# noisystreet/aither

Hardware: AMD Instinct MI355X
Metric: Mcell-updates/sec per iteration (residual+LU-SGS), 256^3 block; % HBM roofline (higher is better)
Workload: dtype f64

## Files before the change

aither_amd/csrc/agx_api.hip:

```cpp
#include "agx_kernels.hpp"
#include "agx_geometry.hpp"
#include "agx_mem.hpp"
#include <rccl/rccl.h>
#include <cstdarg>
#include <cstdio>
#include <cstring>
#include <cstdlib>
#include <cmath>
#include <vector>
#include <string>
#include <algorithm>

using namespace agx;

static char g_err[512] = "";
static int fail(const char* fmt, ...) {
  va_list ap;
  va_start(ap, fmt);
  vsnprintf(g_err, sizeof g_err, fmt, ap);
  va_end(ap);
  return 1;
}
#define HIPCHK(call)                                                       \
  do {                                                                     \
    hipError_t e_ = (call);                                                \
    if (e_ != hipSuccess)                                                  \
      return fail("%s failed: %s (%s:%d)", #call, hipGetErrorString(e_),   \
                  __FILE__, __LINE__);                                     \
  } while (0)
#define AGX_BY_MODE(sp, kernel, grid, block, stream, ...)                                  \
  do {                                                                                     \
    switch (agx::solver_mode_of(sp)) {                                                     \
      case 0: hipLaunchKernelGGL(kernel<0>, grid, block, 0, stream, __VA_ARGS__); break;   \
      case 1: hipLaunchKernelGGL(kernel<1>, grid, block, 0, stream, __VA_ARGS__); break;   \
      default: hipLaunchKernelGGL(kernel<2>, grid, block, 0, stream, __VA_ARGS__); break;  \
    }                                                                                      \
  } while (0)

namespace {

struct SweepGraphs {
  hipGraphExec_t g[2][2][2] = {};
  SweepGraphs() = default;
  SweepGraphs(SweepGraphs&& o) noexcept { memcpy(g, o.g, sizeof g); memset(o.g, 0, sizeof g); }
  ~SweepGraphs() { drop(); }
  hipGraphExec_t& at(bool forward, bool full, bool un_is_u) { return g[forward][full][un_is_u]; }
  void drop() {
    for (auto& g1 : g) for (auto& g2 : g1) for (auto& g3 : g2)
      if (g3) { hipGraphExecDestroy(g3); g3 = nullptr; }
  }
};

struct Block {
  BlockDev d;
  int global_pos = 0;
  DevBuf<double> slab;
  DevBuf<double> d2;
  DevBuf<double> blockmat;
  DevBuf<double> sweep_rec;
  bool sweep_geo_built = false;
  bool x_planes_current = false;
  DevBuf<double> mg_forcing, mg_mres, mg_xsave, mg_nodes;
// ... 64 lines not shown
  DevBuf<NormPartial> partials;
  long n_partials = 0;
  DevBuf<NormPartial> norm_out;
  PinnedBuf<NormPartial> norm_host;
  DevBuf<int> err_dev;
  PinnedBuf<int> err_host;
  DevBuf<double> halo_buf;
  DevBuf<double> stage_buf;
  DevBuf<double> rans_rec;
  bool use_gather = false;
  bool use_tile = true;
  int num_cu = 256;
  bool eager_ghosts = true;
  bool overlap = true;
  hipStream_t ov_stream = nullptr;
  hipEvent_t ov_ready = nullptr, ov_done = nullptr;
  bool visc_gather = false;
  bool visc_march = false;
  int lusgs_mode = 1;
  int spin_limit = 4000000;
  bool allow_fuse = true;
  bool fused_pending = false;
  bool use_graphs = true;
  bool sweep_records = true;
  bool sweep_three = true;
  hipStream_t cap_stream = nullptr;
  std::vector<hipStream_t> branch_streams;
  std::vector<hipEvent_t> branch_events;
  bool sweep_all_launch = true;
  DevBuf<BlockDev> blocks_tab;
  PinnedBuf<BlockDev> blocks_tab_host;
  SweepGraphs sweep_graph_all;
  bool mg_coarse = false;
  bool mres_plane_form = false;
  bool sweep_pipe = true;
  DevBuf<PipeJob> pipe_jobs[2];
  DevBuf<int> pipe_slot0;
  DevBuf<long long> pipe_progress;
  DevBuf<unsigned long long> pipe_ticket;
  size_t pipe_nblocks = 0;
  int pipe_njobs = 0, pipe_maxsteps = 0, pipe_waves = 4;
  long long pipe_launches = 0;
  bool halo_batch = true;
  bool halo_batch_required = false;
  int halo_batch_sides = 0;
  long halo_batch_nmax = 0;
  std::vector<int> halo_conn_order;
  struct HaloLevel { int first, sides; long nmax; };
  std::vector<HaloLevel> halo_levels;
  DevBuf<HaloSide> halo_tab_dev[5][2][2];
  bool halo_tab_valid[5][2] = {};
  int halo_set[5] = {};
  PinnedBuf<HaloSide> halo_tab_host;
  int mresid_split = 1;
  bool mresid_march = true;
  bool have_time_n = false;
  bool have_wall_data = false;
  bool in_iterate = false, ghosts_prefilled = false;
  bool mres_deferred = false;
  hipEvent_t norm_event = nullptr;
  bool consn_pending = false;
  bool state_is_time_n = false;
  long fused_parts = 0;
  bool timing = false;
  std::vector<std::pair<hipEvent_t, hipEvent_t>> ev_pool;
  std::vector<std::pair<int, int>> ev_used;
  double t_ms[G_NGROUP] = {};
  long t_n[G_NGROUP] = {};
};

static int my_side(const agx_ctx* c, const Conn& k);

namespace {

void resolve_timing(agx_ctx* c);

struct Timer {
  agx_ctx* c;
  int slot = -1;
  Timer(agx_ctx* ctx, int g) : c(ctx) {
    if (!c->timing) return;
    if (c->ev_used.size() >= 8192) resolve_timing(c);
    slot = (int)c->ev_used.size();
    if (slot >= (int)c->ev_pool.size()) {
      hipEvent_t a, b;
      if (hipEventCreate(&a) != hipSuccess || hipEventCreate(&b) != hipSuccess) {
        slot = -1;
        return;
      }
      c->ev_pool.emplace_back(a, b);
    }
    c->ev_used.emplace_back(g, slot);
    hipEventRecord(c->ev_pool[slot].first, c->stream);
  }
  ~Timer() {
    if (slot >= 0) hipEventRecord(c->ev_pool[slot].second, c->stream);
  }
};

void resolve_timing(agx_ctx* c) {
  if (c->ev_used.empty()) return;
  hipStreamSynchronize(c->stream);
  for (auto& u : c->ev_used) {
    float ms = 0.f;
    if (hipEventElapsedTime(&ms, c->ev_pool[u.second].first,
                            c->ev_pool[u.second].second) == hipSuccess) {
// ... 150 lines not shown
}

int halo_in_d2(const Block& b, int what) { return what == AGX_HALO_UPDATE && b.d.d2.base ? 1 : 0; }
void x_changed(agx_ctx* c) {
  for (auto& blk : c->blocks) blk.x_planes_current = false;
}
Planes5 halo_planes(Block& b, int what) {
  Planes5 r;
  r.rec = what == AGX_HALO_UPDATE ? b.d.sw_dyn : nullptr;
  const bool z2 = halo_in_d2(b, what) != 0;
  r.stride = z2 ? 2 : 1;
#if AGX_NEQ == 7
  if (what == AGX_HALO_TURB) {
    for (int e = 0; e < AGX_NEQ; ++e) r.p[e] = b.d.turb3[e < 3 ? e : 2];
    return r;
  }
#endif
  if (what == AGX_HALO_VELGRAD_A || what == AGX_HALO_VELGRAD_B) {
    for (int e = 0; e < AGX_NEQ; ++e) {
      const int comp = what == AGX_HALO_VELGRAD_A ? e : std::min(5 + e, 8);
      r.p[e] = b.d.vg + (long)comp * b.d.nplane;
    }
    return r;
  }
  for (int e = 0; e < AGX_NEQ; ++e)
    r.p[e] = what == AGX_HALO_STATE ? b.d.state[e]
             : (z2 ? b.d.d2.base + 2L * (PA_X + (e >> 1)) * b.d.d2.nd2 + (e & 1) : b.d.x[e]);
  return r;
}

int check_device_error(agx_ctx* c) {
  int* const err_host = c->err_host.get();
  if (*err_host) {
    const int code = *err_host;
    *err_host = 0;
    hipMemsetAsync(c->err_dev.get(), 0, sizeof(int), c->stream);
    if (code == 3)
      return fail("Singular matrix in Gauss-Jordan elimination!");
    if (code == AGX_ERR_TPG_ENERGY)
      return fail("thermallyPerfect: the temperature of a cell's specific energy was not "
                  "found (Newton's method did not converge in %d steps, or the energy lies "
                  "below the heat of formation)", AGX_TPG_NEWTON_MAX);
    if (code == 2) {
      c->pipe_nblocks = 0;
      return fail("LU-SGS pipeline: a k-plane waited beyond the spin limit for its "
                  "predecessor (AGX_LUSGS=plane / AGX_SWEEP_PIPE=0 select the "
                  "launch-per-hyperplane forms)");
    }
    return fail("a boundary-condition variant outside this build's coverage was requested");
  }
  return 0;
}

struct MarchPlan { dim3 grid; int kchunk; long nparts; };
int g_march_tj = 6;
bool tile_ok(const agx_ctx* c, const BlockDev& b) {
  return AGX_FAST && c->use_tile && !c->use_gather && (double)b.nplane * 8.0 < 4294967296.0;
}
bool all_tile_ok(const agx_ctx* c) {
  for (const auto& blk : c->blocks)
    if (!tile_ok(c, blk.d)) return false;
  return true;
}
MarchPlan march_plan(const agx_ctx* c, const BlockDev& b) {
  MarchPlan p;
  const int gx = (b.ni + 63) / 64, gy = (b.nj + g_march_tj - 1) / g_march_tj;
  if (tile_ok(c, b)) {
    const long steps = (long)gx * gy * b.nk;
    long np = std::min<long>(c->num_cu, std::max<long>(1, steps / 8));
    if (np >= 8) np -= np % 8;
    p.kchunk = 0;
    p.grid = dim3((unsigned)np);
    p.nparts = np;
    return p;
  }
  int nz = std::max(1, (int)std::lround(2048.0 / (gx * gy)));
  nz = std::min(nz, std::max(1, b.nk / 4));
  p.kchunk = (b.nk + nz - 1) / nz;
  nz = (b.nk + p.kchunk - 1) / p.kchunk;
  p.grid = dim3(gx, gy, nz);
  p.nparts = (long)gx * gy * nz;
  return p;
}

SlabDev make_slab(const BlockDev& b) {
  SlabDev sd;
  sd.base = b.vol - (long)PL_VOL * b.nplane;
  sd.nplane = b.nplane; sd.sx = b.sx; sd.sxy = b.sxy;
  sd.ni = b.ni; sd.nj = b.nj; sd.nk = b.nk; sd.ng = b.ng; sd.ioff = b.ioff;
  sd.st = (int)((b.state[0] - sd.base) / b.nplane);
  sd.sn = (int)((b.state2[0] - sd.base) / b.nplane);
  return sd;
}
template <int RECON, int LIM, int FLUX>
void launch_inv_kernel(agx_ctx* c, const BlockDev& b, double cfl, bool fuse,
                       const MarchArgs& ma, const MarchPlan& mp) {
  const SlabDev sd = make_slab(b);
  if (c->use_gather || AGX_NEQ != 5) {
    hipLaunchKernelGGL((k_inv_residual<RECON, LIM, FLUX>), cell_grid(b, CELL_BLOCK),
                       CELL_BLOCK, 0, c->stream, b, c->gas, c->sp, cfl);
    return;
  }
  const dim3 tb(64, g_march_tj + 2);
#if AGX_FAST
  if (tile_ok(c, b)) {
    if (fuse && ma.store_consn)
      hipLaunchKernelGGL((k_residual_tile<RECON, LIM, FLUX, 2, 6>), mp.grid, tb, 0,
                         c->stream, sd, c->gas, c->sp, cfl, ma);
    else if (fuse)
      hipLaunchKernelGGL((k_residual_tile<RECON, LIM, FLUX, 1, 6>), mp.grid, tb, 0,
                         c->stream, sd, c->gas, c->sp, cfl, ma);
    else
      hipLaunchKernelGGL((k_residual_tile<RECON, LIM, FLUX, 0, 6>), mp.grid, tb, 0,
                         c->stream, sd, c->gas, c->sp, cfl, ma);
  } else
#endif
  {
    if (fuse)
      hipLaunchKernelGGL((k_residual_march<RECON, LIM, FLUX, true, 6>), mp.grid, tb, 0,
                         c->stream, sd, c->gas, c->sp, cfl, ma);
    else
      hipLaunchKernelGGL((k_residual_march<RECON, LIM, FLUX, false, 6>), mp.grid, tb, 0,
                         c->stream, sd, c->gas, c->sp, cfl, ma);
  }
}
template <int RECON, int LIM>
// ... 829 lines not shown
  }
#if AGX_FAST
  for (auto& b : c->blocks)
    if (b.d.d2.base) {
      const long n = (long)b.d.d2.Pi * b.d.d2.Pj * (b.d.nk + 2 * b.d.ng);
      hipLaunchKernelGGL(k_d2_geo, dim3((n + 255) / 256), dim3(256), 0, c->stream, b.d);
    }
  HIPCHK(hipGetLastError());
#endif
  HIPCHK(hipStreamSynchronize(c->stream));
  for (auto& b : c->blocks) {
    b.fcen.reset();
    b.nodes_dev.reset();
  }
  return 0;
}
}

extern "C" {

const char* agx_last_error(void) { return g_err; }
const char* agx_version(void) {
#if AGX_TPG
  return "aither_gfx950 0.1 (HIP, gfx950, thermallyPerfect)";
#else
  return "aither_gfx950 0.1 (HIP, gfx950)";
#endif
}

int agx_ctx_create(int device, int rank, agx_ctx** out) {
  int ndev = 0;
  hipError_t e = hipGetDeviceCount(&ndev);
  if (e != hipSuccess || ndev <= 0)
    return fail("no HIP device available (%s): the gfx950 library has no CPU "
                "path", hipGetErrorString(e));
  if (device < 0 || device >= ndev) return fail("device %d out of range", device);
  HIPCHK(hipSetDevice(device));
  agx_ctx* c = new agx_ctx();
  c->device = device;
  c->rank = rank;
  if (const char* kn = getenv("AGX_KERNEL")) {
    c->use_gather = !strcmp(kn, "gather");
    c->use_tile = !strcmp(kn, "tile");
  }
  c->allow_fuse = !(getenv("AGX_NO_FUSE") && atoi(getenv("AGX_NO_FUSE")) != 0);
  {
    int ncu = 0;
    HIPCHK(hipDeviceGetAttribute(&ncu, hipDeviceAttributeMultiprocessorCount, device));
    if (ncu > 0) c->num_cu = ncu;
    if (const char* w = getenv("AGX_WORKGROUPS")) c->num_cu = std::max(1, atoi(w));
    if (const char* w = getenv("AGX_VISC")) {
      c->visc_gather = !strcmp(w, "gather");
      c->visc_march = !strcmp(w, "march");
    }
    if (const char* w = getenv("AGX_EAGER_GHOSTS")) c->eager_ghosts = atoi(w) != 0;
    if (const char* w = getenv("AGX_OVERLAP")) c->overlap = atoi(w) != 0;
    if (const char* w = getenv("AGX_LUSGS")) c->lusgs_mode = !strcmp(w, "plane") ? 0 : 1;
    if (const char* w = getenv("AGX_SPIN_LIMIT")) c->spin_limit = std::max(1, atoi(w));
    if (const char* w = getenv("AGX_GRAPHS")) c->use_graphs = atoi(w) != 0;
    if (const char* w = getenv("AGX_SWEEP_ALL")) c->sweep_all_launch = atoi(w) != 0;
    if (const char* w = getenv("AGX_SWEEP_PIPE")) c->sweep_pipe = atoi(w) != 0;
    if (const char* w = getenv("AGX_SWEEP_THREE")) c->sweep_three = atoi(w) != 0;
    if (const char* w = getenv("AGX_SWEEP_RECORDS")) c->sweep_records = atoi(w) != 0;
    if (const char* w = getenv("AGX_MRESID_SPLIT")) c->mresid_split = std::min(64, std::max(1, atoi(w)));
    if (const char* w = getenv("AGX_MRESID")) c->mresid_march = strcmp(w, "plane") != 0;
    if (const char* w = getenv("AGX_HALO_BATCH")) {
      c->halo_batch = strcmp(w, "0") != 0;
      c->halo_batch_required = !strcmp(w, "require");
    }
  }
  HIPCHK(c->err_dev.alloc(1));
  HIPCHK(hipMemset(c->err_dev.get(), 0, sizeof(int)));
  HIPCHK(c->err_host.alloc(1));
  *c->err_host.get() = 0;
  *out = c;
  return 0;
}

void agx_ctx_destroy(agx_ctx* c) {
  if (!c) return;
  hipSetDevice(c->device);
  hipStreamSynchronize(c->stream);
  if (c->nccl) ncclCommDestroy(c->nccl);
  for (auto& e : c->ev_pool) { hipEventDestroy(e.first); hipEventDestroy(e.second); }
  if (c->cap_stream) hipStreamDestroy(c->cap_stream);
  if (c->ov_stream) {
    hipStreamSynchronize(c->ov_stream);
    hipStreamDestroy(c->ov_stream);
    hipEventDestroy(c->ov_ready);
    hipEventDestroy(c->ov_done);
  }
  for (auto ev : c->branch_events) hipEventDestroy(ev);
  for (auto st : c->branch_streams) hipStreamDestroy(st);
  delete c;
}

int agx_ctx_set_stream(agx_ctx* c, void* s) {
  HIPCHK(hipSetDevice(c->device));
  HIPCHK(hipStreamSynchronize(c->stream));
  c->stream = (hipStream_t)s;
  return 0;
}

int agx_config_set(agx_ctx* c, const agx_config* cfg) {
  if (!c->blocks.empty())
    return fail("agx_config_set: the configuration is fixed after the first "
// ... 1042 lines not shown
  hipLaunchKernelGGL(k_mg_nodes, dim3((bc.d.ni + tb.x) / tb.x, (bc.d.nj + tb.y) / tb.y, bc.d.nk + 1),
                     tb, 0, cz->stream, bc.d, bc.mg_nodes.get());
  HIPCHK(hipGetLastError());
  if (mg_order(cz, f)) return 1;
  hipLaunchKernelGGL(k_mg_prolong, cell_grid(bf.d, tb), tb, 0, f->stream, bf.d, m,
                     (const double*)bc.mg_nodes.get(), bc.d.ni, bc.d.nj, bc.d.nk);
  mg_x_records(cz, bc);
  mg_x_records(f, bf);
  if (mg_x_from_planes(cz, bc) || mg_x_from_planes(f, bf)) return 1;
  HIPCHK(hipGetLastError());
  return 0;
}

int agx_store_time_n(agx_ctx* c, int also_nm1) {
  if (flush_consn(c)) return 1;
  c->have_time_n = true;
  for (auto& blk : c->blocks)
    if (blk.nr_max > 0) c->ghosts_prefilled = false;
  static const bool lazy = !(getenv("AGX_NO_LAZY_CONSN") && atoi(getenv("AGX_NO_LAZY_CONSN")));
  c->state_is_time_n = true;
  if (lazy && !also_nm1 && !c->use_gather && all_tile_ok(c)) { c->consn_pending = true; return 0; }
  for (auto& blk : c->blocks)
    hipLaunchKernelGGL(k_store_time_n, cell_grid(blk.d, CELL_BLOCK), CELL_BLOCK,
                       0, c->stream, blk.d, c->gas, also_nm1);
  HIPCHK(hipGetLastError());
  return 0;
}

int agx_phase_bc_faces(agx_ctx* c) { Timer t(c, G_BC); return bc_pass(c, true, 0); }
int agx_phase_bc_edges(agx_ctx* c) { Timer t(c, G_BC); return bc_pass(c, false, 0); }

int agx_phase_residual(agx_ctx* c, int mm, double cfl) {
  if (c->cfg.dt_nondim <= 0.0 && cfl <= 0.0)
    return fail("Neither dt or cfl was specified!");
  c->sp.diag_add = c->mg_coarse ? 1 : 0;
  const bool fuse = can_fuse(c);
  const int store_consn = !c->use_gather && all_tile_ok(c) && c->consn_pending && mm == 0;
  if (store_consn) c->consn_pending = false;
  else if (flush_consn(c)) return 1;
  {
    Timer t(c, G_RESID);
    long off = 0;
    for (auto& blk : c->blocks) {
      const MarchPlan mp = march_plan(c, blk.d);
      MarchArgs ma;
      memset(&ma, 0, sizeof ma);
      ma.kchunk = mp.kchunk;
      ma.mode = c->cfg.time_integration == AGX_TIME_RK4 ? 1 : 0;
      ma.store_consn = store_consn;
      const double rk_alpha[4] = {0.25, 1.0 / 3.0, 0.5, 1.0};
      ma.alpha = rk_alpha[mm & 3];
      ma.partials = c->partials.get() + off;
      ma.ablate = getenv("AGX_ABLATE") ? atoi(getenv("AGX_ABLATE")) : 0;
      launch_inv(c, blk.d, cfl, fuse, ma, mp);
      off += mp.nparts;
      if (c->sp.implicit && c->sp.block) launch_block_diag(c, blk.d);
    }
  }
  HIPCHK(hipGetLastError());
  c->fused_pending = fuse;
  if (c->cfg.is_viscous) {
    {
      Timer t(c, G_BC);
      if (bc_pass(c, true, 1)) return 1;
      if (bc_pass(c, false, 1)) return 1;
      c->have_wall_data = true;
    }
    Timer t(c, G_VISC);
    for (auto& blk : c->blocks)
#if AGX_NEQ == 7
      {
        const int fourth = c->cfg.viscous_recon == AGX_VISC_RECON_CENTRAL_4TH ? 1 : 0;
        const BlockDev& vb = blk.d;
        if (c->visc_gather) {
          hipLaunchKernelGGL(k_visc_residual_rans, cell_grid(vb, CELL_BLOCK), CELL_BLOCK,
                             0, c->stream, vb, c->gas, c->sp, cfl, fourth);
          continue;
        }
        RansRec rec;
        rec.ni1 = vb.ni + 1; rec.nj1 = vb.nj + 1;
        rec.nf = (long)rec.ni1 * rec.nj1 * (vb.nk + 1);
        const size_t need = (size_t)3 * RANS_REC * rec.nf;
        if (need > c->rans_rec.size()) {
          HIPCHK(hipStreamSynchronize(c->stream));
          HIPCHK(c->rans_rec.alloc(need));
        }
        rec.p = c->rans_rec.get();
        const dim3 tb = CELL_BLOCK;
        auto fgrid = [&](int di, int dj, int dk) {
          return dim3((vb.ni + di + tb.x - 1) / tb.x, (vb.nj + dj + tb.y - 1) / tb.y, vb.nk + dk);
        };
        hipLaunchKernelGGL(k_rans_faces<0>, fgrid(1, 0, 0), tb, 0, c->stream, vb, c->gas, fourth, rec);
        hipLaunchKernelGGL(k_rans_faces<1>, fgrid(0, 1, 0), tb, 0, c->stream, vb, c->gas, fourth, rec);
        hipLaunchKernelGGL(k_rans_faces<2>, fgrid(0, 0, 1), tb, 0, c->stream, vb, c->gas, fourth, rec);
        hipLaunchKernelGGL(k_rans_cells, cell_grid(vb, tb), tb, 0, c->stream, vb, c->gas, c->sp,
                           cfl, fourth, rec);
      }
#else
    {
      const bool fourth = c->cfg.viscous_recon == AGX_VISC_RECON_CENTRAL_4TH;
      const bool wide_plane = (double)blk.d.nplane * 8.0 >= 4294967296.0;
      if (!AGX_FAST || c->visc_gather || (fourth && (c->visc_march || wide_plane))) {
        hipLaunchKernelGGL(k_visc_residual, cell_grid(blk.d, CELL_BLOCK), CELL_BLOCK,
                           0, c->stream, blk.d, c->gas, c->sp, cfl, fourth ? 1 : 0);
      } else {
        const BlockDev& vb = blk.d;
        if (c->visc_march || wide_plane) {
          const int gx = (vb.ni + VTI - 1) / VTI, gy = (vb.nj + VTJ - 1) / VTJ;
          int nz = std::max(1, std::min(vb.nk / 8, (int)std::lround(2048.0 / (gx * gy))));
          const int kchunk = (vb.nk + nz - 1) / nz;
          nz = (vb.nk + kchunk - 1) / kchunk;
          hipLaunchKernelGGL(k_visc_march, dim3(gx, gy, nz), dim3(64, VTJ + 1), 0, c->stream,
                             vb, c->gas, c->sp, cfl, kchunk);
          continue;
        }
#if AGX_FAST
        const int oi = fourth ? VT_L - 4 : VT_OI;
        const int gx = (vb.ni + oi - 1) / oi, gy = (vb.nj + VT_OJ - 1) / VT_OJ;
        const long steps = (long)gx * gy * vb.nk;
        const int nwg = (int)std::min<long>(c->num_cu, std::max<long>(1, steps / 8));
        if (fourth)
          hipLaunchKernelGGL(k_visc_tile<true>, dim3(nwg), dim3(VT_L, VT_R), 0, c->stream,
                             make_slab(vb), c->gas, c->sp, cfl, gx, gy);
        else
          hipLaunchKernelGGL(k_visc_tile<false>, dim3(nwg), dim3(VT_L, VT_R), 0, c->stream,
                             make_slab(vb), c->gas, c->sp, cfl, gx, gy);
#endif
      }
    }
#endif
#if AGX_NEQ != 7
    if (c->sp.implicit && c->sp.block)
      for (auto& blk : c->blocks)
        hipLaunchKernelGGL(k_block_diag_visc, cell_grid(blk.d, CELL_BLOCK), CELL_BLOCK, 0,
                           c->stream, blk.d, c->gas, c->sp,
                           c->cfg.viscous_recon == AGX_VISC_RECON_CENTRAL_4TH ? 1 : 0);
#endif
    HIPCHK(hipGetLastError());
  }
  for (auto& blk : c->blocks)
    if (blk.nr_max > 0) {
      Timer t(c, G_BC);
      hipLaunchKernelGGL(k_nr_grads, dim3((blk.nr_max + 255) / 256, blk.d.nsurf), dim3(256), 0,
                         c->stream, blk.d, c->gas);
      HIPCHK(hipGetLastError());
    }
  return 0;
}

int agx_phase_explicit_update(agx_ctx* c, int mm, double* l2, agx_linf* linf) {
  const int mode = c->cfg.time_integration == AGX_TIME_RK4 ? 1 : 0;
  return update_pass(c, mode, mm, l2, linf);
}

static int implicit_begin(agx_ctx* c, int write_x);
#if AGX_FAST
static void d2_prepare(agx_ctx* c, Block& blk, int write_x, int again) {
  const BlockDev& b = blk.d;
  const dim3 grid((b.d2.Pi + TT - 1) / TT, (b.d2.Pj + TT - 1) / TT, b.nk + 2 * b.ng);
  hipLaunchKernelGGL(k_lusgs_prepare, grid, dim3(256), 0, c->stream, b, c->gas, c->sp,
                     write_x, write_x ? (unsigned)(++blk.kp_epoch) & 3u : 0u, again);
}
#endif
int agx_phase_implicit_begin(agx_ctx* c) { return implicit_begin(c, 1); }
static int implicit_begin(agx_ctx* c, int write_x) {
  x_changed(c);
  Timer t(c, G_PREPARE);
  c->sp.un_is_u = c->state_is_time_n ? 1 : 0;
  for (auto& blk : c->blocks) {
    const BlockDev& b = blk.d;
#if AGX_FAST
    if (b.d2.base) {
      bool conn = false;
      for (int q = 0; q < 6; ++q) conn = conn || b.side_conn[q] != 0;
      d2_prepare(c, blk, write_x && (c->sp.requires_init || conn) ? 1 : 0, 0);
      continue;
    }
#endif
    if (!c->sp.requires_init && write_x)
// ... 460 lines not shown
```

aither_amd/csrc/agx_kernels.hpp:

```cpp
#pragma once
#include "agx_device.hpp"
#include "agx_lusgs.hpp"

namespace agx {

struct BlockDev {
  int ni, nj, nk, ng;
  int ioff;
  long sx, sxy, nplane;
  int parent;
  double* state[AGX_NEQ];
  double* state2[AGX_NEQ];
  double* fa[3][4];
  double* vol;
  double* cen[3];
  double* wid[3];
  double* resid[AGX_NEQ];
  double* specrad;
  double* dt;
  double* consn[AGX_NEQ];
  double* consnm1[AGX_NEQ];
  double* x[AGX_NEQ];
  double* xold[AGX_NEQ];
  double* a;
  double* ainv;
  double* am;
  double* aminv;
  double* vg;
  double* specrad_t;
  double* a_t;
  double* ainv_t;
  double* viscp;
  double* turb3[3];
  double* am_t;
  double* aminv_t;
  double* wdist;
  double* sw_geo;
  double* sw_dyn;
  double* sw_rhs;
  double* mg_forcing;
  double* mg_mres;
  double* mg_xsave;
  D2Dev d2;
  const agx_bc_surface* surf;
  int nsurf, nsurf_i, nsurf_j, nsurf_k;
  const int* nr_off;
  double* nr_grad;
  const int* wall_off;
  WallVars* wallv;
  double* nr_mach;
  int side_conn[6];
  __host__ __device__ long idx(int i, int j, int k) const {
    return (long)(k + ng) * sxy + (long)(j + ng) * sx + (i + ioff);
  }
  __host__ __device__ long stride(int d) const {
// ... 163 lines not shown
  const int i = blockIdx.x * blockDim.x + threadIdx.x;
  const int j = blockIdx.y * blockDim.y + threadIdx.y;
  const int k = blockIdx.z;
  if (i >= b.ni || j >= b.nj) return;
  constexpr int H = RECON == AGX_RECON_CONSTANT ? 1
                    : (RECON == AGX_RECON_MUSCL ? 2 : 3);
  constexpr int NS = 2 * H + 1;
  const long q = b.idx(i, j, k);
  double res[AGX_NEQ] = {0.0, 0.0, 0.0, 0.0, 0.0};
  double sr = 0.0, srt = 0.0;
#pragma unroll
  for (int d = 0; d < 3; ++d) {
    const long s = b.stride(d);
    double st[NS][AGX_NEQ], w[NS];
#pragma unroll
    for (int m = 0; m < NS; ++m) {
      const long qq = q + (m - H) * s;
      load5(b.state, qq, st[m]);
      w[m] = b.wid[d][qq];
    }
    double al[4], au[4], f[AGX_NEQ];
    load_area(b, d, q, al);
    load_area(b, d, q + s, au);
    face_flux_1d<RECON, LIM, FLUX>(g, sp.kappa, st, w, H, al, f);
#pragma unroll
    for (int e = 0; e < AGX_NEQ; ++e) res[e] -= f[e] * al[3];
    face_flux_1d<RECON, LIM, FLUX>(g, sp.kappa, st, w, H + 1, au, f);
#pragma unroll
    for (int e = 0; e < AGX_NEQ; ++e) res[e] += f[e] * au[3];
    sr += inv_cell_spec_rad(g, st[H], al, au);
    if (AGX_NEQ > 5) {
      const double v[3] = {0.5 * (al[0] + au[0]), 0.5 * (al[1] + au[1]), 0.5 * (al[2] + au[2])};
      srt += fabs(dot3(st[H] + 1, v)) * fast_rsqrt(dot3(v, v)) * (0.5 * (al[3] + au[3]));
    }
  }
  store5(b.resid, q, res);
  b.specrad[q] = sr;
  if (sp.implicit) b.a[q] = sp.diag_add ? b.a[q] + sr : sr;
  if (AGX_NEQ > 5) {
    b.specrad_t[q] = srt;
    if (sp.implicit) b.a_t[q] = sp.diag_add ? b.a_t[q] + srt : srt;
  }
  if (!sp.viscous)
    b.dt[q] = sp.dt_fixed > 0.0 ? sp.dt_fixed : cfl * (b.vol[q] / fmax(sr, 0.0));
}

struct MarchArgs {
  int kchunk;
  int mode;
  double alpha;
  int store_consn;
  int ablate;
  NormPartial* partials;
};

template <int RECON, int LIM>
__device__ __forceinline__ void recon_face(const SlabDev& b, int d, long qc,
                                           long s, double kappa, double* l,
                                           double* r) {
  if (RECON == AGX_RECON_CONSTANT) {
#pragma unroll
    for (int e = 0; e < AGX_NEQ; ++e) { l[e] = b.state(e)[qc - s]; r[e] = b.state(e)[qc]; }
  } else if (RECON == AGX_RECON_MUSCL) {
    const double* wd = b.wid(d);
    const double w2 = wd[qc - 2 * s], w1 = wd[qc - s], w0 = wd[qc], wp = wd[qc + s];
    const double r10 = fast_rcp(w1 + w0);
    const double dPl = (w1 + w1) * r10, dMl = (w1 + w1) * fast_rcp(w1 + w2);
    const double dPr = (w0 + w0) * r10, dMr = (w0 + w0) * fast_rcp(w0 + wp);
#pragma unroll
    for (int e = 0; e < AGX_NEQ; ++e) {
      const double* p = b.state(e);
      const double u2 = p[qc - 2 * s], u1 = p[qc - s], u0 = p[qc], up = p[qc + s];
      l[e] = muscl<LIM>(u2, u1, u0, dPl, dMl, kappa);
      r[e] = muscl<LIM>(up, u0, u1, dPr, dMr, kappa);
    }
  } else {
    double w[6];
#pragma unroll
    for (int m = 0; m < 6; ++m) w[m] = b.wid(d)[qc + (m - 3) * s];
    const double cwl[5] = {w[0], w[1], w[2], w[3], w[4]};
    const double cwr[5] = {w[5], w[4], w[3], w[2], w[1]};
    WenoCoeffs kl, kr;
    weno_coeffs(cwl, kl);
    weno_coeffs(cwr, kr);
#pragma unroll
    for (int e = 0; e < AGX_NEQ; ++e) {
      const double* p = b.state(e);
      double u[6];
#pragma unroll
      for (int m = 0; m < 6; ++m) u[m] = p[qc + (m - 3) * s];
      l[e] = weno<RECON == AGX_RECON_WENOZ>(kl, u[0], u[1], u[2], u[3], u[4]);
      r[e] = weno<RECON == AGX_RECON_WENOZ>(kr, u[5], u[4], u[3], u[2], u[1]);
    }
  }
}
template <int RECON, int LIM, int FLUX>
__device__ __forceinline__ void face_flux_area(const SlabDev& b, const GasDev& g,
                                               double kappa, int d, long qc,
                                               long s, const double* area,
                                               double* f) {
  double l[AGX_NEQ], r[AGX_NEQ];
  recon_face<RECON, LIM>(b, d, qc, s, kappa, l, r);
  inviscid_flux<FLUX>(g, l, r, area, f);
#pragma unroll
  for (int e = 0; e < AGX_NEQ; ++e) f[e] *= area[3];
}

// ... 194 lines not shown
    }
  } else {
    {
      double cw[5];
#pragma unroll
      for (int m = 0; m < 5; ++m) cw[m] = getw(m - 3);
      WenoCoeffs kc;
      weno_coeffs(cw, kc);
#pragma unroll
      for (int e = 0; e < AGX_NEQ; ++e)
        l[e] = weno<RECON == AGX_RECON_WENOZ>(kc, get(e, -3), get(e, -2), get(e, -1),
                                              get(e, 0), get(e, 1));
    }
    AGX_SB_SIDES;
    {
      double cw[5];
#pragma unroll
      for (int m = 0; m < 5; ++m) cw[m] = getw(2 - m);
      WenoCoeffs kc;
      weno_coeffs(cw, kc);
#pragma unroll
      for (int e = 0; e < AGX_NEQ; ++e)
        r[e] = weno<RECON == AGX_RECON_WENOZ>(kc, get(e, 2), get(e, 1), get(e, 0),
                                              get(e, -1), get(e, -2));
    }
  }
}

template <int RECON, int LIM, int FLUX, int FUSE, int TJ>
__global__ void __launch_bounds__(64 * (TJ + 2), 2)
k_residual_tile(SlabDev b, GasDev g, SolverDev sp, double cfl, MarchArgs ma) {
  constexpr int H = RECON == AGX_RECON_CONSTANT ? 1
                    : (RECON == AGX_RECON_MUSCL ? 2 : 3);
  constexpr bool BAL = TJ >= 4;
  constexpr int NV = AGX_NEQ + 2;
  constexpr int TW = 64 + 2 * H, TR = TJ + 2 * H;
  constexpr int PLANE = TR * TW;
  __shared__ double tile[2][NV][TR][TW];
  __shared__ double sFj[2][TJ + 1][AGX_NEQ][64];
  __shared__ double sFi[2][TJ][AGX_NEQ];
  constexpr bool PARK = H <= 2;
  __shared__ double sNorm[AGX_NEQ + 1][TJ][64];
  __shared__ long long sLin[TJ][64];
  __shared__ double sFk[PARK ? TJ : 1][AGX_NEQ][64];
  __shared__ double sAk[PARK ? TJ : 1][4][64];
  const int lane = threadIdx.x, wv = threadIdx.y;
  const long s_k = b.sxy;
  if (FUSE && wv < TJ) {
#pragma unroll
    for (int e = 0; e < AGX_NEQ; ++e) sNorm[e][wv][lane] = 0.0;
    sNorm[AGX_NEQ][wv][lane] = -1.0e300;
    sLin[wv][lane] = 0x7fffffffffffffffLL;
  }
  const int gx = (b.ni + 63) / 64, gy = (b.nj + TJ - 1) / TJ;
  const long S = (long)gx * gy * b.nk;
  const int P = gridDim.x;
  const int rr = P % 8 == 0 ? (int)(blockIdx.x % 8) * (P / 8) + (int)(blockIdx.x / 8)
                            : (int)blockIdx.x;
  long s_pos = S * rr / P;
  const long s_end = S * (rr + 1) / P;
  while (s_pos < s_end) {
  const int col = (int)(s_pos / b.nk);
  const int k0 = (int)(s_pos - (long)col * b.nk);
  const int k1 = (int)min((long)b.nk, k0 + (s_end - s_pos));
  s_pos += k1 - k0;
  const int i0 = (col % gx) * 64, j0 = (col / gx) * TJ;
  const int itop = min(i0 + 64, b.ni), jtop = min(j0 + TJ, b.nj);
  if (wv < TJ) {
    const int i = i0 + lane, j = j0 + wv;
    const bool cell = i < itop && j < jtop;
    const int ic = min(i, b.ni + b.ng - 1), jc = min(j, b.nj + b.ng - 1);
    long q = b.idx(ic, jc, k0);
    const int to = (wv + H) * TW + lane + H;
    const int pw = PARK ? wv : 0;
    double W[2 * H][AGX_NEQ], wk[2 * H];
    double fk_reg[AGX_NEQ] = {0, 0, 0, 0, 0}, ak_reg[4];
    {
      double W0[AGX_NEQ], w0, ak_lo[4], fk_lo[AGX_NEQ] = {0, 0, 0, 0, 0};
      b.area(2, q, ak_lo);
#pragma unroll
      for (int e = 0; e < AGX_NEQ; ++e) W0[e] = b.state(e)[q - H * s_k];
      w0 = b.wid(2)[q - H * s_k];
#pragma unroll
      for (int m = 0; m < 2 * H; ++m) {
#pragma unroll
        for (int e = 0; e < AGX_NEQ; ++e) W[m][e] = b.state(e)[q + (m - H + 1) * s_k];
        wk[m] = b.wid(2)[q + (m - H + 1) * s_k];
      }
      if (cell) {
        double l[AGX_NEQ], r[AGX_NEQ];
        recon_generic<RECON, LIM>(
            [&](int e, int m) { return m + H == 0 ? W0[e] : W[m + H - 1][e]; },
            [&](int m) { return m + H == 0 ? w0 : wk[m + H - 1]; }, sp.kappa, l, r);
        inviscid_flux<FLUX>(g, l, r, ak_lo, fk_lo);
#pragma unroll
        for (int e = 0; e < AGX_NEQ; ++e) fk_lo[e] *= ak_lo[3];
      }
      if (PARK) {
#pragma unroll
        for (int e = 0; e < AGX_NEQ; ++e) sFk[pw][e][lane] = fk_lo[e];
#pragma unroll
        for (int e = 0; e < 4; ++e) sAk[pw][e][lane] = ak_lo[e];
      } else {
#pragma unroll
        for (int e = 0; e < AGX_NEQ; ++e) fk_reg[e] = fk_lo[e];
#pragma unroll
        for (int e = 0; e < 4; ++e) ak_reg[e] = ak_lo[e];
      }
      double* tl = &tile[0][0][0][0];
#pragma unroll
      for (int e = 0; e < AGX_NEQ; ++e) tl[e * PLANE + to] = W[H - 1][e];
      tl[AGX_NEQ * PLANE + to] = b.wid(0)[q];
      tl[(AGX_NEQ + 1) * PLANE + to] = b.wid(1)[q];
    }
    __syncthreads();
    int cur = 0;
    unsigned qb = (unsigned)(q * 8);
    const unsigned skb = (unsigned)(s_k * 8), sxb = (unsigned)(b.sx * 8);
// ... 159 lines not shown
        if (i == itop - 1) {
#pragma unroll
          for (int e = 0; e < AGX_NEQ; ++e) res[e] += sFi[cur][wv][e];
        }
        const double sr = (sr_i + sr_j) + sr_k;
        const double dt = sp.dt_fixed > 0.0 ? sp.dt_fixed
                                            : cfl * (vol * fast_rcp(fmax(sr, 0.0)));
        const bool st_ok = !AGX_AB(4) || res[0] == 12345.678;
        if (st_ok) {
#pragma unroll
          for (int e = 0; e < AGX_NEQ; ++e) b.stb(PL_RESID + e, qb, res[e]);
          b.stb(PL_SPECRAD, qb, sr);
          if (sp.implicit) b.stb(PL_A, qb, sp.diag_add ? b.ldb(PL_A, qb) + sr : sr);
          if (!sp.viscous) b.stb(PL_DT, qb, dt);
          if (FUSE == 0 && ma.store_consn) {
            double u0[AGX_NEQ];
            prim_to_cons(g, sc, u0);
#pragma unroll
            for (int e = 0; e < AGX_NEQ; ++e) b.stb(PL_CONSN + e, qb, u0[e]);
          }
        }
        if (FUSE) {
          double u[AGX_NEQ], ns[AGX_NEQ];
          double fac = dt * fast_rcp(vol);
          if (ma.mode == 0 || FUSE == 2) {
            prim_to_cons(g, sc, u);
            if (FUSE == 2 && st_ok) {
#pragma unroll
              for (int e = 0; e < AGX_NEQ; ++e) b.stb(PL_CONSN + e, qb, u[e]);
            }
          } else {
#pragma unroll
            for (int e = 0; e < AGX_NEQ; ++e) u[e] = cn[e];
          }
          if (ma.mode != 0) fac *= ma.alpha;
#pragma unroll
          for (int e = 0; e < AGX_NEQ; ++e) u[e] -= fac * res[e];
          if AGX_AB(8) {
#pragma unroll
            for (int e = 0; e < AGX_NEQ; ++e) ns[e] = u[e];
          } else {
            cons_to_prim(g, u, ns);
          }
          if (st_ok) {
#pragma unroll
            for (int e = 0; e < AGX_NEQ; ++e) b.stb(b.sn + e, qb, ns[e]);
          }
          const long lin0 = (((long)k * b.nj + j) * b.ni + i) * AGX_NEQ;
          double vm = sNorm[AGX_NEQ][wv][lane];
          long long vl = sLin[wv][lane];
#pragma unroll
          for (int e = 0; e < AGX_NEQ; ++e) {
            sNorm[e][wv][lane] += res[e] * res[e];
            if (res[e] > vm) { vm = res[e]; vl = lin0 + e; }
          }
          sNorm[AGX_NEQ][wv][lane] = vm;
          sLin[wv][lane] = vl;
        }
      }
#pragma unroll
      for (int m = 0; m < 2 * H - 1; ++m) {
#pragma unroll
        for (int e = 0; e < AGX_NEQ; ++e) W[m][e] = W[m + 1][e];
        wk[m] = wk[m + 1];
      }
#pragma unroll
      for (int e = 0; e < AGX_NEQ; ++e) W[2 * H - 1][e] = nxt[e];
      wk[2 * H - 1] = nwk;
    }
  } else {
    const bool top = wv == TJ;
    const int gi = min(i0 + lane, b.ni + b.ng - 1);
    long qrow[H];
    int lrow[H];
#pragma unroll
    for (int m = 0; m < H; ++m) {
      const int row = top ? TJ + H + m : m;
      const int gj = min(max(j0 - H + row, -b.ng), b.nj + b.ng - 1);
      qrow[m] = b.idx(gi, gj, 0);
      lrow[m] = row * TW + lane + H;
    }
    const bool hc = !top && lane < 2 * H * TJ;
    const int cc = lane % (2 * H), crow = H + min(lane / (2 * H), TJ - 1);
    const int ccol = cc < H ? cc : 64 + cc;
    const long qcol = b.idx(min(max(i0 - H + ccol, -b.ng), b.ni + b.ng - 1),
                            min(j0 - H + crow, b.nj + b.ng - 1), 0);
    const int lcol = crow * TW + ccol;
    bool do_f;
    long qf;
    int fo;
    if (top) {
      do_f = i0 + lane < itop;
      qf = b.idx(min(i0 + lane, b.ni), jtop, 0);
      fo = (jtop - j0 + H) * TW + lane + H;
    } else {
      do_f = lane < TJ && j0 + lane < jtop;
      qf = b.idx(itop, min(j0 + lane, b.nj), 0);
      fo = (min(lane, TJ - 1) + H) * TW + (itop - i0) + H;
    }
    {
      double* tl = &tile[0][0][0][0];
#pragma unroll
      for (int v = 0; v < NV; ++v) {
        const double* p = b.pl(v < AGX_NEQ ? b.st + v : PL_WID + (v - AGX_NEQ));
#pragma unroll
        for (int m = 0; m < H; ++m) tl[v * PLANE + lrow[m]] = p[qrow[m] + (long)k0 * s_k];
        if (hc) tl[v * PLANE + lcol] = p[qcol + (long)k0 * s_k];
// ... 2566 lines not shown
```

aither_amd/csrc/agx_visc_tile.hpp:

```cpp
#pragma once

namespace agx {

constexpr int VT_L = 64, VT_R = 8;
constexpr int VT_OI = VT_L - 2, VT_OJ = VT_R - 2;
enum { VS_S0 = 0, VS_SM = 4, VS_SP = 8, VS_AI0 = 12, VS_AJ0 = 15, VS_AJ1 = 18, VS_AK0 = 21,
       VS_AK1 = 24, VS_VOL = 27, VS_WJ = 28, VS_RHO = 29, VS_MU = 30, VS_AI1 = 31, VS_WI = 34,
       VS_FJ = 35, VS_COUNT = 39 };

#ifndef VT_LDSAREA
#define VT_LDSAREA 1
#endif
#ifndef VT_EDGE_BARRIER
#define VT_EDGE_BARRIER __builtin_amdgcn_sched_barrier(0)
#endif
struct VRef { int var, row, lane; };
using VShared = double (*)[VT_L][VS_COUNT];
__device__ __forceinline__ void vt_ld4(VShared sh, const VRef& r, double* o) {
#pragma unroll
  for (int c = 0; c < 4; ++c) o[c] = sh[r.row][r.lane][r.var + c];
}
__device__ __forceinline__ void vt_ld3(VShared sh, const VRef& r, double* o) {
#pragma unroll
  for (int c = 0; c < 3; ++c) o[c] = sh[r.row][r.lane][r.var + c];
}
__device__ __forceinline__ void vt_acc(double (*grad)[4], const double* val, const double* a,
                                       double sg) {
#pragma unroll
  for (int r = 0; r < 3; ++r) {
    const double w = sg * a[r];
#pragma unroll
    for (int c = 0; c < 4; ++c) grad[r][c] = fma(val[c], w, grad[r][c]);
  }
}
struct VtEdge { VRef c0, c1, a0, a1; };
__device__ __forceinline__ void vt_edge(VShared sh, double (*grad)[4], const double* vsum,
                                        const VtEdge& e, double sg) {
  double c0[4], c1[4], a0[3], a1[3], v[4], a[3];
  vt_ld4(sh, e.c0, c0); vt_ld4(sh, e.c1, c1);
  vt_ld3(sh, e.a0, a0); vt_ld3(sh, e.a1, a1);
#pragma unroll
  for (int c = 0; c < 4; ++c) v[c] = 0.25 * (vsum[c] + c0[c] + c1[c]);
#pragma unroll
  for (int r = 0; r < 3; ++r) a[r] = 0.5 * (a0[r] + a1[r]);
  vt_acc(grad, v, a, sg);
  VT_EDGE_BARRIER;
}
struct VtNoWide {
  __device__ __forceinline__ void operator()(double*, double*, double&, double&) const {}
};
template <bool F4, class Wide>
__device__ __forceinline__ void vt_face(VShared sh, const GasDev& g, const VRef& rL,
                                        const VRef& rU, const VRef& rhoL, const VRef& rhoU,
                                        double rhoU_reg, double muU_reg, bool u_in_reg,
                                        const double* uReg, const double* aF, const double* aFm,
                                        const double* aFp, const VtEdge& t1u, const VtEdge& t1l,
                                        const VtEdge& t2u, const VtEdge& t2l, double volL,
                                        double volU, double wL, double wU, double* f,
// ... 32 lines not shown
    for (int c = 0; c < 4; ++c) grad[r][c] *= inv_vol;
  const double rL_ = sh[rhoL.row][rhoL.lane][rhoL.var];
  const double mL_ = sh[rhoL.row][rhoL.lane][rhoL.var + 1];
  const double rU_ = u_in_reg ? rhoU_reg : sh[rhoU.row][rhoU.lane][rhoU.var];
  const double mU_ = u_in_reg ? muU_reg : sh[rhoU.row][rhoU.lane][rhoU.var + 1];
  double vf[3], tf, mu;
  if constexpr (F4) {
    double c0[6], c3[6], w0 = 1.0, w3 = 1.0;
    wide(c0, c3, w0, w3);
    const double w1 = wL, w2 = wU;
    const double r01 = fast_rcp(w0 + w1), r12 = fast_rcp(w1 + w2), r23 = fast_rcp(w2 + w3);
    const double t012 = fast_rcp(w0 + w1 + w2), t123 = fast_rcp(w1 + w2 + w3);
    const double q4 = fast_rcp((w0 + w1) + (w2 + w3));
    const double k3 = w1 * w2, k4 = k3 * (w0 + w1);
    auto c4 = [&](double u0, double u1, double u2, double u3) {
      const double g01 = (u1 - u0) * r01, g12 = (u2 - u1) * r12, g23 = (u3 - u2) * r23;
      const double d3a = (g12 - g01) * t012, d3b = (g23 - g12) * t123;
      return u1 + w1 * g12 - k3 * d3a - k4 * ((d3b - d3a) * q4);
    };
#pragma unroll
    for (int c = 0; c < 3; ++c) vf[c] = c4(c0[c], vL[c], vU[c], c3[c]);
    const double rf = c4(c0[4], rL_, rU_, c3[4]);
    const double pf = c4(c0[4] * c0[3], rL_ * vL[3], rU_ * vU[3], c3[4] * c3[3]);
    tf = pf * fast_rcp(rf);
    mu = g.scaling * c4(c0[5], mL_, mU_, c3[5]);
  } else {
    const double iw = fast_rcp(wL + wU);
    const double cD = wU * iw, cU = wL * iw;
#pragma unroll
    for (int c = 0; c < 3; ++c) vf[c] = cD * vU[c] + cU * vL[c];
    const double rf = cD * rU_ + cU * rL_;
    tf = (cD * rU_ * vU[3] + cU * rL_ * vL[3]) * fast_rcp(rf);
    mu = g.scaling * (cD * mU_ + cU * mL_);
  }
  const double lambda = -(2.0 / 3.0) * mu;
  const double trace = grad[0][0] + grad[1][1] + grad[2][2];
  double tau[3];
#pragma unroll
  for (int r = 0; r < 3; ++r) {
    const double mm = (grad[r][0] + grad[0][r]) * aF[0] + (grad[r][1] + grad[1][r]) * aF[1] +
                      (grad[r][2] + grad[2][r]) * aF[2];
    tau[r] = lambda * trace * aF[r] + mu * mm;
  }
  const double kk = conductivity(g, tf) * g.scaling;
  const double tg = grad[0][3] * aF[0] + grad[1][3] * aF[1] + grad[2][3] * aF[2];
  f[0] = tau[0];
  f[1] = tau[1];
  f[2] = tau[2];
  f[3] = dot3(tau, vf) + kk * tg;
}

template <bool F4>
__global__ void __launch_bounds__(VT_L * VT_R)
k_visc_tile(SlabDev b, GasDev g, SolverDev sp, double cfl, int gx, int gy) {
  __shared__ double sh[VT_R][VT_L][VS_COUNT];
  constexpr int LO = F4 ? 2 : 1;
  constexpr int OI = F4 ? VT_L - 4 : VT_OI;
  const int l = threadIdx.x, ty = threadIdx.y;
  const long S = (long)gx * gy * b.nk;
  const int P = gridDim.x;
  const int rr = P % 8 == 0 ? (int)(blockIdx.x % 8) * (P / 8) + (int)(blockIdx.x / 8)
                            : (int)blockIdx.x;
  long s_pos = S * rr / P;
  const long s_end = S * (rr + 1) / P;
  while (s_pos < s_end) {
  const int col = (int)(s_pos / b.nk);
  const int k0 = (int)(s_pos - (long)col * b.nk);
  const int k1 = (int)min((long)b.nk, k0 + (s_end - s_pos));
  s_pos += k1 - k0;
  const int ci = (col % gx) * OI - LO + l, cj = (col / gx) * VT_OJ - 1 + ty;
  const bool inner = l >= LO && l < LO + OI && ty >= 1 && ty <= VT_OJ;
  const bool own = inner && ci < b.ni && cj < b.nj;
  const bool do_i = l >= LO && l <= LO + OI && ty >= 1 && ty <= VT_OJ && ci <= b.ni && cj < b.nj;
  const bool do_j = ty >= 1 && l >= LO && l < LO + OI && cj <= b.nj && ci < b.ni;
  const int ic = min(ci, F4 ? b.ni + 1 : b.ni), jc = min(cj, F4 ? b.nj + 1 : b.nj);
  const unsigned qc = (unsigned)(b.idx(ic, jc, 0) * 8);
  const unsigned sk = (unsigned)(b.sxy * 8), sj = (unsigned)(b.sx * 8);
  const int kcmax = b.nk + b.ng - 1, kfmax = b.nk + b.ng;
  auto ld_state = [&](int k, double* s4, double& rho, double& mu) {
    const unsigned q = qc + (unsigned)min(k, kcmax) * sk;
    rho = b.ldb(b.st + 0, q);
    s4[0] = b.ldb(b.st + 1, q); s4[1] = b.ldb(b.st + 2, q); s4[2] = b.ldb(b.st + 3, q);
    s4[3] = rho > 0.0 ? b.ldb(b.st + 4, q) * fast_rcp(rho * g.R) : 0.0;
    mu = rho > 0.0 ? viscosity(g, s4[3]) : 0.0;
  };
  auto rq_state = [&](int k, double* raw) {
    const unsigned q = qc + (unsigned)min(k, kcmax) * sk;
#pragma unroll
    for (int e = 0; e < 5; ++e) raw[e] = b.ldb(b.st + e, q);
  };
  auto cv_state = [&](const double* raw, double* s4, double& rho, double& mu) {
    rho = raw[0];
    s4[0] = raw[1]; s4[1] = raw[2]; s4[2] = raw[3];
    s4[3] = rho > 0.0 ? raw[4] * fast_rcp(rho * g.R) : 0.0;
    mu = rho > 0.0 ? viscosity(g, s4[3]) : 0.0;
  };
  auto ld_avec = [&](int d, unsigned q, double* a3) {
    const double mag = b.ldb(PL_FA + 4 * d + 3, q);
    a3[0] = b.ldb(PL_FA + 4 * d + 0, q) * mag; a3[1] = b.ldb(PL_FA + 4 * d + 1, q) * mag;
    a3[2] = b.ldb(PL_FA + 4 * d + 2, q) * mag;
  };
  auto rq_avec = [&](int d, unsigned q, double* raw) {
#pragma unroll
    for (int c = 0; c < 4; ++c) raw[c] = b.ldb(PL_FA + 4 * d + c, q);
  };
  auto cv_avec = [&](const double* raw, double* a3) {
    a3[0] = raw[0] * raw[3]; a3[1] = raw[1] * raw[3]; a3[2] = raw[2] * raw[3];
  };
  auto PUT4 = [&](int var, const double* v) {
#pragma unroll
    for (int c = 0; c < 4; ++c) sh[ty][l][var + c] = v[c];
  };
  auto PUT3 = [&](int var, const double* v) {
#pragma unroll
    for (int c = 0; c < 3; ++c) sh[ty][l][var + c] = v[c];
  };
  auto LD4 = [&](int var, int row, int lane, double* o) {
#pragma unroll
    for (int c = 0; c < 4; ++c) o[c] = sh[row][lane][var + c];
  };
  auto LD3 = [&](int var, int row, int lane, double* o) {
#pragma unroll
// ... 219 lines not shown
```

Before: 1457.

## Add step-ordered tile plan to balance k-march segments across workgroups

Introduces a host-computed TilePlan that splits the tile×k iteration space into k-chunks ordered step-wise across tiles, charging each segment restart with the halo warm-up cost, and uses it in the inviscid and viscous tiled march kernels. The goal is to balance per-workgroup work, including the restart overhead of reloading halo planes, rather than splitting the flat column-major range evenly. Plans are cached per shape, and the column ordering can still be selected through an environment variable. The change adds per-segment index arithmetic inside the kernels and may produce more segment restarts, each of which reloads halo planes.

After: 1479 (median of 6 runs). 1.5% higher.

```diff
diff --git a/aither_amd/csrc/agx_api.hip b/aither_amd/csrc/agx_api.hip
--- a/aither_amd/csrc/agx_api.hip
+++ b/aither_amd/csrc/agx_api.hip
@@ -8,6 +8,8 @@
 #include <cstdlib>
 #include <cmath>
 #include <vector>
+#include <array>
+#include <map>
 #include <string>
 #include <algorithm>
 
@@ -178,6 +180,9 @@
   bool halo_tab_valid[5][2] = {};
   int halo_set[5] = {};
   PinnedBuf<HaloSide> halo_tab_host;
+  int tile_order_inv = TILE_ORDER_STEP;
+  int tile_order_visc = TILE_ORDER_STEP;
+  std::map<std::array<int, 6>, TilePlan> tile_plans;
   int mresid_split = 1;
   bool mresid_march = true;
   bool have_time_n = false;
@@ -434,7 +439,7 @@
   return 0;
 }
 
-struct MarchPlan { dim3 grid; int kchunk; long nparts; };
+struct MarchPlan { dim3 grid; int kchunk; long nparts; TilePlan tile; };
 int g_march_tj = 6;
 bool tile_ok(const agx_ctx* c, const BlockDev& b) {
   return AGX_FAST && c->use_tile && !c->use_gather && (double)b.nplane * 8.0 < 4294967296.0;
@@ -444,9 +449,17 @@
     if (!tile_ok(c, blk.d)) return false;
   return true;
 }
-MarchPlan march_plan(const agx_ctx* c, const BlockDev& b) {
+TilePlan tile_plan_of(agx_ctx* c, int gx, int gy, int nk, int P, int charge, int order) {
+  const std::array<int, 6> key = {gx, gy, nk, P, charge, order};
+  auto it = c->tile_plans.find(key);
+  if (it == c->tile_plans.end())
+    it = c->tile_plans.emplace(key, tile_plan_make(gx, gy, nk, P, charge, order)).first;
+  return it->second;
+}
+MarchPlan march_plan(agx_ctx* c, const BlockDev& b) {
   MarchPlan p;
-  const int gx = (b.ni + 63) / 64, gy = (b.nj + g_march_tj - 1) / g_march_tj;
+  const int gx = tile_count(b.ni, TILE_INV_I), gy = tile_count(b.nj, g_march_tj);
+  p.tile = tile_plan_column(gx * gy, b.nk);
   if (tile_ok(c, b)) {
     const long steps = (long)gx * gy * b.nk;
     long np = std::min<long>(c->num_cu, std::max<long>(1, steps / 8));
@@ -454,6 +467,8 @@
     p.kchunk = 0;
     p.grid = dim3((unsigned)np);
     p.nparts = np;
+    const int halo = c->cfg.recon == AGX_RECON_CONSTANT ? 1 : (c->cfg.recon == AGX_RECON_MUSCL ? 2 : 3);
+    p.tile = tile_plan_of(c, gx, gy, b.nk, (int)np, tile_charge_inviscid(halo), c->tile_order_inv);
     return p;
   }
   int nz = std::max(1, (int)std::lround(2048.0 / (gx * gy)));
@@ -1389,6 +1404,13 @@
     if (const char* w = getenv("AGX_VISC")) {
       c->visc_gather = !strcmp(w, "gather");
       c->visc_march = !strcmp(w, "march");
+    }
+    if (const char* w = getenv("AGX_TILE_ORDER")) {
+      if (strcmp(w, "step") && strcmp(w, "column")) {
+        delete c;
+        return fail("AGX_TILE_ORDER is '%s': step or column", w);
+      }
+      c->tile_order_inv = c->tile_order_visc = !strcmp(w, "step") ? TILE_ORDER_STEP : TILE_ORDER_COLUMN;
     }
     if (const char* w = getenv("AGX_EAGER_GHOSTS")) c->eager_ghosts = atoi(w) != 0;
     if (const char* w = getenv("AGX_OVERLAP")) c->overlap = atoi(w) != 0;
@@ -2537,6 +2559,7 @@
       ma.alpha = rk_alpha[mm & 3];
       ma.partials = c->partials.get() + off;
       ma.ablate = getenv("AGX_ABLATE") ? atoi(getenv("AGX_ABLATE")) : 0;
+      ma.plan = mp.tile;
       launch_inv(c, blk.d, cfl, fuse, ma, mp);
       off += mp.nparts;
       if (c->sp.implicit && c->sp.block) launch_block_diag(c, blk.d);
@@ -2600,16 +2623,19 @@
           continue;
         }
 #if AGX_FAST
-        const int oi = fourth ? VT_L - 4 : VT_OI;
-        const int gx = (vb.ni + oi - 1) / oi, gy = (vb.nj + VT_OJ - 1) / VT_OJ;
+        const int gx = tile_count(vb.ni, fourth ? TILE_VISC_I_F4 : TILE_VISC_I);
+        const int gy = tile_count(vb.nj, TILE_J);
         const long steps = (long)gx * gy * vb.nk;
         const int nwg = (int)std::min<long>(c->num_cu, std::max<long>(1, steps / 8));
+        const TilePlan tp = tile_plan_of(c, gx, gy, vb.nk, nwg,
+                                         fourth ? TILE_CHARGE_VISC_F4 : TILE_CHARGE_VISC,
+                                         c->tile_order_visc);
         if (fourth)
           hipLaunchKernelGGL(k_visc_tile<true>, dim3(nwg), dim3(VT_L, VT_R), 0, c->stream,
-                             make_slab(vb), c->gas, c->sp, cfl, gx, gy);
+                             make_slab(vb), c->gas, c->sp, cfl, gx, tp);
         else
           hipLaunchKernelGGL(k_visc_tile<false>, dim3(nwg), dim3(VT_L, VT_R), 0, c->stream,
-                             make_slab(vb), c->gas, c->sp, cfl, gx, gy);
+                             make_slab(vb), c->gas, c->sp, cfl, gx, tp);
 #endif
       }
     }
diff --git a/aither_amd/csrc/agx_kernels.hpp b/aither_amd/csrc/agx_kernels.hpp
--- a/aither_amd/csrc/agx_kernels.hpp
+++ b/aither_amd/csrc/agx_kernels.hpp
@@ -1,6 +1,7 @@
 #pragma once
 #include "agx_device.hpp"
 #include "agx_lusgs.hpp"
+#include "agx_tile_plan.hpp"
 
 namespace agx {
 
@@ -270,7 +271,23 @@
   int store_consn;
   int ablate;
   NormPartial* partials;
+  TilePlan plan;
 };
+
+__device__ __forceinline__ TileWalk tile_walk_begin(const TilePlan& p) {
+  const int P = gridDim.x;
+  TileWalk w = tile_plan_range(p, tile_range_of((int)blockIdx.x, P), P);
+  w.v = __builtin_amdgcn_readfirstlane(w.v); w.v1 = __builtin_amdgcn_readfirstlane(w.v1);
+  return w;
+}
+__device__ __forceinline__ bool tile_walk_next(const TilePlan& p, TileWalk& w, TileSeg& s) {
+  const bool more = tile_plan_next(p, w, s);
+  w.v = __builtin_amdgcn_readfirstlane(w.v);
+  s.col = __builtin_amdgcn_readfirstlane(s.col);
+  s.k0 = __builtin_amdgcn_readfirstlane(s.k0);
+  s.k1 = __builtin_amdgcn_readfirstlane(s.k1);
+  return __builtin_amdgcn_readfirstlane((int)more) != 0;
+}
 
 template <int RECON, int LIM>
 __device__ __forceinline__ void recon_face(const SlabDev& b, int d, long qc,
@@ -571,18 +588,11 @@
     sNorm[AGX_NEQ][wv][lane] = -1.0e300;
     sLin[wv][lane] = 0x7fffffffffffffffLL;
   }
-  const int gx = (b.ni + 63) / 64, gy = (b.nj + TJ - 1) / TJ;
-  const long S = (long)gx * gy * b.nk;
-  const int P = gridDim.x;
-  const int rr = P % 8 == 0 ? (int)(blockIdx.x % 8) * (P / 8) + (int)(blockIdx.x / 8)
-                            : (int)blockIdx.x;
-  long s_pos = S * rr / P;
-  const long s_end = S * (rr + 1) / P;
-  while (s_pos < s_end) {
-  const int col = (int)(s_pos / b.nk);
-  const int k0 = (int)(s_pos - (long)col * b.nk);
-  const int k1 = (int)min((long)b.nk, k0 + (s_end - s_pos));
-  s_pos += k1 - k0;
+  const int gx = tile_count(b.ni, TILE_INV_I);
+  TileWalk walk = tile_walk_begin(ma.plan);
+  TileSeg seg;
+  while (tile_walk_next(ma.plan, walk, seg)) {
+  const int col = seg.col, k0 = seg.k0, k1 = seg.k1;
   const int i0 = (col % gx) * 64, j0 = (col / gx) * TJ;
   const int itop = min(i0 + 64, b.ni), jtop = min(j0 + TJ, b.nj);
   if (wv < TJ) {
@@ -848,7 +858,7 @@
 #pragma unroll
           for (int e = 0; e < AGX_NEQ; ++e) {
             sNorm[e][wv][lane] += res[e] * res[e];
-            if (res[e] > vm) { vm = res[e]; vl = lin0 + e; }
+            if (res[e] > vm || (res[e] == vm && lin0 + e < vl)) { vm = res[e]; vl = lin0 + e; }
           }
           sNorm[AGX_NEQ][wv][lane] = vm;
           sLin[wv][lane] = vl;
diff --git a/aither_amd/csrc/agx_tile_plan.hpp b/aither_amd/csrc/agx_tile_plan.hpp
--- /dev/null
+++ b/aither_amd/csrc/agx_tile_plan.hpp
@@ -0,0 +1,100 @@
+#pragma once
+
+#if defined(__HIPCC__)
+#define AGX_TP_HD __host__ __device__
+#else
+#define AGX_TP_HD
+#endif
+
+namespace agx {
+
+enum { TILE_ORDER_COLUMN = 0, TILE_ORDER_STEP = 1 };
+
+constexpr int TILE_CHARGE_VISC = 3;
+constexpr int TILE_CHARGE_VISC_F4 = 5;
+AGX_TP_HD inline int tile_charge_inviscid(int halo) { return 2 * halo; }
+
+constexpr int TILE_INV_I = 64, TILE_VISC_I = 62, TILE_VISC_I_F4 = 60, TILE_J = 6;
+AGX_TP_HD inline int tile_count(int n, int owned) { return (n + owned - 1) / owned; }
+
+struct TilePlan {
+  int tiles;
+  int nk;
+  int L;
+  int c;
+};
+struct TileSeg { int col, k0, k1; };
+struct TileWalk { int v, v1; };
+
+AGX_TP_HD inline int tile_plan_chunks(const TilePlan& p) { return (p.nk + p.L - 1) / p.L; }
+AGX_TP_HD inline long tile_plan_span(const TilePlan& p) {
+  return (long)p.tiles * (p.nk + (long)p.c * tile_plan_chunks(p));
+}
+AGX_TP_HD inline bool tile_plan_is_column(const TilePlan& p) { return p.c == 0 && p.L == p.nk; }
+AGX_TP_HD inline TilePlan tile_plan_column(int tiles, int nk) { return TilePlan{tiles, nk, nk, 0}; }
+
+AGX_TP_HD inline int tile_range_of(int wg, int P) {
+  return P % 8 == 0 ? (wg % 8) * (P / 8) + wg / 8 : wg;
+}
+AGX_TP_HD inline int tile_xcd_of_range(int r, int P) { return P % 8 == 0 ? r / (P / 8) : -1; }
+
+AGX_TP_HD inline TileWalk tile_plan_range(const TilePlan& p, int r, int P) {
+  const long V = tile_plan_span(p);
+  return TileWalk{(int)(V * r / P), (int)(V * (r + 1) / P)};
+}
+AGX_TP_HD inline bool tile_plan_next(const TilePlan& p, TileWalk& w, TileSeg& s) {
+  const int full = p.tiles * (p.L + p.c);
+  while (w.v < w.v1) {
+    const int m = w.v / full;
+    const int kb = m * p.L;
+    const int Lm = p.L < p.nk - kb ? p.L : p.nk - kb;
+    const int run = (w.v - m * full) / (Lm + p.c);
+    const int rs = m * full + run * (Lm + p.c);
+    const int o = w.v - rs - p.c, e = w.v1 - rs - p.c;
+    const int ks = o > 0 ? o : 0, ke = e < Lm ? e : Lm;
+    w.v = rs + Lm + p.c < w.v1 ? rs + Lm + p.c : w.v1;
+    if (ke > ks) {
+      s.col = run; s.k0 = kb + ks; s.k1 = kb + ke;
+      return true;
+    }
+  }
+  return false;
+}
+
+inline long tile_plan_cost(const TilePlan& p, int P, int charge) {
+  long worst = 0;
+  for (int r = 0; r < P; ++r) {
+    TileWalk w = tile_plan_range(p, r, P);
+    TileSeg s;
+    long cost = 0;
+    while (tile_plan_next(p, w, s)) cost += (s.k1 - s.k0) + charge;
+    if (cost > worst) worst = cost;
+  }
+  return worst;
+}
+
+inline TilePlan tile_plan_make(int gx, int gy, int nk, int P, int charge, int order) {
+  const int tiles = gx * gy;
+  const TilePlan column = tile_plan_column(tiles, nk);
+  if (order != TILE_ORDER_STEP || tiles < 2 || P < 8 || nk < 2) return column;
+  if ((long)tiles * nk * (1 + charge) > 0x7fffffffL) return column;
+  int L = 0;
+  if (tiles > P) {
+    const long S = (long)tiles * nk, q = (S + P - 1) / P, runs = (q + nk - 1) / nk;
+    L = (int)((q + runs - 1) / runs);
+  } else {
+    long best = -1;
+    for (int l = 1; l < nk; ++l) {
+      const long d = (long)(l + charge) * P - tile_plan_span(TilePlan{tiles, nk, l, charge});
+      const long ad = d < 0 ? -d : d;
+      if (best < 0 || ad < best) { best = ad; L = l; }
+    }
+    if (best > P) return column;
+  }
+  if (L < 1 || L >= nk) return column;
+  const TilePlan step{tiles, nk, L, charge};
+  if (tile_plan_cost(step, P, charge) > tile_plan_cost(column, P, charge) + charge) return column;
+  return step;
+}
+
+}
diff --git a/aither_amd/csrc/agx_visc_tile.hpp b/aither_amd/csrc/agx_visc_tile.hpp
--- a/aither_amd/csrc/agx_visc_tile.hpp
+++ b/aither_amd/csrc/agx_visc_tile.hpp
@@ -1,9 +1,12 @@
 #pragma once
+#include "agx_tile_plan.hpp"
 
 namespace agx {
 
 constexpr int VT_L = 64, VT_R = 8;
 constexpr int VT_OI = VT_L - 2, VT_OJ = VT_R - 2;
+static_assert(VT_OI == TILE_VISC_I && VT_L - 4 == TILE_VISC_I_F4 && VT_OJ == TILE_J,
+              "the plan's tile sizes (agx_tile_plan.hpp) are this kernel's");
 enum { VS_S0 = 0, VS_SM = 4, VS_SP = 8, VS_AI0 = 12, VS_AJ0 = 15, VS_AJ1 = 18, VS_AK0 = 21,
        VS_AK1 = 24, VS_VOL = 27, VS_WJ = 28, VS_RHO = 29, VS_MU = 30, VS_AI1 = 31, VS_WI = 34,
        VS_FJ = 35, VS_COUNT = 39 };
@@ -142,22 +145,15 @@
 
 template <bool F4>
 __global__ void __launch_bounds__(VT_L * VT_R)
-k_visc_tile(SlabDev b, GasDev g, SolverDev sp, double cfl, int gx, int gy) {
+k_visc_tile(SlabDev b, GasDev g, SolverDev sp, double cfl, int gx, TilePlan tp) {
   __shared__ double sh[VT_R][VT_L][VS_COUNT];
   constexpr int LO = F4 ? 2 : 1;
   constexpr int OI = F4 ? VT_L - 4 : VT_OI;
   const int l = threadIdx.x, ty = threadIdx.y;
-  const long S = (long)gx * gy * b.nk;
-  const int P = gridDim.x;
-  const int rr = P % 8 == 0 ? (int)(blockIdx.x % 8) * (P / 8) + (int)(blockIdx.x / 8)
-                            : (int)blockIdx.x;
-  long s_pos = S * rr / P;
-  const long s_end = S * (rr + 1) / P;
-  while (s_pos < s_end) {
-  const int col = (int)(s_pos / b.nk);
-  const int k0 = (int)(s_pos - (long)col * b.nk);
-  const int k1 = (int)min((long)b.nk, k0 + (s_end - s_pos));
-  s_pos += k1 - k0;
+  TileWalk walk = tile_walk_begin(tp);
+  TileSeg seg;
+  while (tile_walk_next(tp, walk, seg)) {
+  const int col = seg.col, k0 = seg.k0, k1 = seg.k1;
   const int ci = (col % gx) * OI - LO + l, cj = (col / gx) * VT_OJ - 1 + ty;
   const bool inner = l >= LO && l < LO + OI && ty >= 1 && ty <= VT_OJ;
   const bool own = inner && ci < b.ni && cj < b.nj;
```
